# tue-mps/simple-tad

Measured on AMD Instinct MI355X. Metric: clips/sec (16x224^2 ViT-B) fwd+bwd, higher is better.
Workload: dtype bf16; 1 GPU; vit_base_patch16_224 16x224x224, 32 clips/GPU, fwd+bwd+AdamW fine-tune step with CE loss on synthetic labels (BASELINE configs[2]/[3]); global_batch=32, per_gpu_batch=32, parallelism=dp1, residual_stream=f32, operands=bf16, parameters=86228738

## Files before the change

simple_tad_amd/csrc/gemm.hip:

```cpp
#include <math.h>
#include <stdlib.h>
#include <string>
#include "common.h"

TAD_NAMESPACE_BEGIN

int launch_reduce_partials(const float* partial, float* out, int splits, int64_t n, int accumulate, hipStream_t st);
int launch_reduce_col_ranges(const float* partial, int N, int splits, int c0, float* out0, int c1, float* out1, int n, int accumulate,
                             hipStream_t st);
int launch_reduce_dw(const float* partial, float* out, int splits, int64_t n, int accumulate, const float* partial2, int rows2, int n2,
                     float* out2a, float* out2b, int n2a, int c2b, hipStream_t st);
int launch_reduce_dw_pair(const float* partial, float* outA, float* outB, int64_t nA, int splits, int64_t n, int accumulate, const float* partial2,
                          int rows2, int n2, float* out2a, float* out2b, int n2a, int c2b, hipStream_t st);

#ifdef TAD_GEMM_ABLATION
#define DBG_BITS(p) ((p).debug)
#else
#define DBG_BITS(p) 0
#endif

enum { EPI_PLAIN = 0, EPI_GELU = 1, EPI_RESIDUAL = 2, EPI_DGELU = 3, EPI_RESMOD = 4 };

struct GemmNT {
  const uint16_t* A;
  const uint16_t* B;
  void* C;
  const float* bias;
  const float* bias2;
  int bias_seg;
  float colscale;
  int colscale_cols;
  const float* residual;
  const float* gamma;
  const float* rowscale;
// ... 831 lines not shown
                                                 c_rs, ob, 0, ST_AUX);
        }
      }
    }
    if (q < 6) { STAMP(5 + 2 * q); }
    if (q + 1 < NCHUNK) lds_barrier();
  }
#undef DROP_CHUNK
  }
  STAMP(2);
#ifdef TAD_GEMM_ABLATION
  if (p.stamps) {
    asm volatile("s_waitcnt vmcnt(0)" ::: "memory");
    STAMP(3);
  }
  ++stamp_i;
#endif
  if (!has_next) break;
  if (!DIRECT) lds_barrier();
  }
}

struct GemmTN {
  const uint16_t* P;
  const uint16_t* Q;
  float* slab;
  float* bias_slab;
  int Mr, N, K;
  int rows_per_split;
  int debug;
  const uint16_t* P2;
  const uint16_t* Q2;
  int N1;
};

__device__ __forceinline__ int sw_tn(int row) { return ((row & 3) | ((row >> 1) & 4)) << 1; }


template <int BM, int BN, int WAVES_M, int WAVES_N, int STAGES, bool PDEEP = false>
__global__ __launch_bounds__(WAVES_M* WAVES_N * 64) void gemm_tn_kernel(const GemmTN p) {
  static_assert(!PDEEP || STAGES == 2, "PDEEP extends the two-stage ring");
  constexpr int BKT = BK;
  constexpr int NW = WAVES_M * WAVES_N;
  constexpr int WTM = BM / WAVES_M, WTN = BN / WAVES_N;
  constexpr int MREP = WTM / 16, NREP = WTN / 16;
  constexpr int PROW = BM * 2, QROW = BN * 2;
  constexpr int KSTEPS = BKT / 32;
  constexpr int P_BYTES = BKT * PROW, Q_BYTES = BKT * QROW;
  constexpr int STAGE_BYTES = P_BYTES + Q_BYTES;
  constexpr int P_PIECES = P_BYTES / 1024 / NW, Q_PIECES = Q_BYTES / 1024 / NW;
  constexpr int P_LPR = PROW / 16, Q_LPR = QROW / 16;
  static_assert(P_BYTES % (1024 * NW) == 0 && Q_BYTES % (1024 * NW) == 0, "tile must split into 1-KiB DMA pieces per wave");
  static_assert(P_LPR <= 64 && Q_LPR <= 64 && PROW >= 256 && QROW >= 256, "row length");
  constexpr int LOADS = P_PIECES + Q_PIECES;
  constexpr int LDS_BYTES_TN = PDEEP ? 3 * P_BYTES + 2 * Q_BYTES : STAGES * STAGE_BYTES;
  static_assert(LDS_BYTES_TN <= 160 * 1024, "LDS budget");
  __shared__ __attribute__((aligned(1024))) char lds[LDS_BYTES_TN];

  const int tid = threadIdx.x;
  const int lane = tid & 63;
  const int wave = __builtin_amdgcn_readfirstlane(tid >> 6);
  const int wm = wave / WAVES_N, wn = wave % WAVES_N;

  const int tiles_k = (p.K + BN - 1) / BN;
  const int tiles = tiles_k * ((p.N + BM - 1) / BM);
  const int lin = xcd_remap(blockIdx.x, gridDim.x);
// ... 161 lines not shown
      const int k = k0 + wn * WTN + 16 * j + 4 * g;
      if (n < p.N && k < p.K)
        *reinterpret_cast<float4*>(out + (int64_t)n * p.K + k) = make_float4(acc[i][j][0], acc[i][j][1], acc[i][j][2], acc[i][j][3]);
    }
  }
}

#ifndef TAD_GEMM_W4_TU

static int cu_count();

TAD_NAMESPACE_END
namespace tad { namespace knobs {
#ifndef TAD_OPND_F16
static int env_int(const char* name) {
  const char* v = getenv(name);
  return v ? atoi(v) : 0;
}
int gemm_debug = env_int("TAD_GEMM_DEBUG");
int nt_persist = !env_int("TAD_GEMM_NO_PERSIST");
int nt_direct = getenv("TAD_GEMM_DIRECT_EPI") ? env_int("TAD_GEMM_DIRECT_EPI") : 1;
int nt_split = getenv("TAD_GEMM_SPLIT_TAIL") ? env_int("TAD_GEMM_SPLIT_TAIL") : 1;
int nt_sk_defer = getenv("TAD_GEMM_SPLITK_DEFER") ? env_int("TAD_GEMM_SPLITK_DEFER") : 1;
int nt_splitk = getenv("TAD_GEMM_SPLITK_TAIL") ? env_int("TAD_GEMM_SPLITK_TAIL") : 1;
int nt_variant = env_int("TAD_GEMM_NT_VARIANT");
int nt_group_m_knob = getenv("TAD_GEMM_GROUP_M") ? env_int("TAD_GEMM_GROUP_M") : 0;
int tn_variant = env_int("TAD_GEMM_TN_VARIANT");
int nt_w4_plain = getenv("TAD_GEMM_W4_PLAIN") ? env_int("TAD_GEMM_W4_PLAIN") : 640;
int nt_w4_epilogues = getenv("TAD_GEMM_W4_EPILOGUES") ? env_int("TAD_GEMM_W4_EPILOGUES") : 4;
int tn_pair = getenv("TAD_GEMM_TN_PAIR") ? env_int("TAD_GEMM_TN_PAIR") : 1;
int nt_short_k = getenv("TAD_GEMM_SHORT_K") ? env_int("TAD_GEMM_SHORT_K") : 1;
int nt_tail_192 = getenv("TAD_GEMM_TAIL_192") ? env_int("TAD_GEMM_TAIL_192") : 1;
int tn_w4 = getenv("TAD_GEMM_TN_W4") ? env_int("TAD_GEMM_TN_W4") : 1;
int tn_pdeep = env_int("TAD_GEMM_TN_PDEEP");
unsigned long long* nt_stamps = nullptr;
long long nt_launches = 0;
#else
extern int gemm_debug, nt_persist, nt_direct, nt_split, nt_splitk, nt_variant, nt_group_m_knob, tn_variant, tn_pdeep, nt_sk_defer, tn_w4, nt_w4_plain, nt_w4_epilogues, nt_tail_192, nt_short_k, tn_pair;
extern unsigned long long* nt_stamps;
extern long long nt_launches;
#endif
}}
TAD_NAMESPACE_BEGIN
using namespace knobs;

static int nt_group_m(int tiles_m, int tiles_n, int K) {
  if (nt_group_m_knob > 0) return nt_group_m_knob;
  return K >= 2048 ? 4 : 8;
}


template <int EPI, bool OUT_BF16>
static void launch_nt_variant(int v, GemmNT& p, hipStream_t st) {
  auto tiles = [&](int bm, int bn) { return ((p.M + bm - 1) / bm) * ((p.N + bn - 1) / bn); };
  const int no_persist = !nt_persist;
  if (((EPI == EPI_RESIDUAL && OUT_BF16) || EPI == EPI_RESMOD) && (v == 1 || v == 7)) v = 3;
  if (v != 2 && v != 4 && v != 5 && p.rowscale && p.rows_per_scale < 256) v = 2;
  const int grid_p = cu_count() & ~7;
  const int bn = v == 1 ? 256 : 128;
  const bool persist = !no_persist && (v == 1 || v == 3) && grid_p >= 8 && tiles(256, bn) > grid_p + grid_p / 2;
  p.group_m = nt_group_m((p.M + 255) / 256, (p.N + bn - 1) / bn, p.K);
#define NT_LAUNCH(BM_, BN_, WM_, WN_, ST_, PER_, DIR_, GRID_, THREADS_)                                                              \
  hipLaunchKernelGGL((gemm_nt_kernel<BM_, BN_, WM_, WN_, ST_, EPI, OUT_BF16, PER_, DIR_>), dim3(GRID_), dim3(THREADS_), 0, st, p)
  const bool direct = nt_direct == 2 || (nt_direct == 1 && EPI == EPI_PLAIN && OUT_BF16);
  switch (v) {
    case 1:
      if constexpr (!(EPI == EPI_RESIDUAL && OUT_BF16) && EPI != EPI_RESMOD) {
        if (persist) { if (direct) NT_LAUNCH(256, 256, 2, 4, 2, true, true, grid_p, 512); else NT_LAUNCH(256, 256, 2, 4, 2, true, false, grid_p, 512); }
        else { if (direct) NT_LAUNCH(256, 256, 2, 4, 2, false, true, tiles(256, 256), 512); else NT_LAUNCH(256, 256, 2, 4, 2, false, false, tiles(256, 256), 512); }
      }
      break;
// ... 266 lines not shown
  return (K > 0 && pad256 * 3 >= pad128 * 4) ? 3 : 1;
}
static int cu_count() {
  static const int n = [] {
    int dev = 0, v = 0;
    if (hipGetDevice(&dev) != hipSuccess || hipDeviceGetAttribute(&v, hipDeviceAttributeMultiprocessorCount, dev) != hipSuccess || v <= 0) v = 256;
    return v;
  }();
  return n;
}
static int tn_plan(int64_t Mr, int N, int K, int* splits, int* rows_per_split) {
  const int bn = tn_variant(K) != 3 ? 256 : 128;
  const int tiles = ((N + 255) / 256) * ((K + bn - 1) / bn);
  const int64_t ktiles = (Mr + BK - 1) / BK;
  const int cus = cu_count();
  const double epi_units = 6.0;
  const double reduce_units = (double)N * (double)K * 8.0 / 4.0e12 / 2.0e-6;
  int best = 1;
  double best_cost = 1e300;
  for (int s = 1; s <= 64 && s <= ktiles; ++s) {
    const int64_t per = (ktiles + s - 1) / s;
    const int s_eff = (int)((ktiles + per - 1) / per);
    if (s_eff != s) continue;
    const int64_t rounds = ((int64_t)tiles * s + cus - 1) / cus;
    const double cost = (double)rounds * ((double)per + epi_units) + (s > 1 ? s * reduce_units : 0.0);
    if (cost < best_cost) { best_cost = cost; best = s; }
  }
  const int64_t per = (ktiles + best - 1) / best;
  *splits = best;
  *rows_per_split = (int)(per * BK);
  return tiles;
}

size_t gemm_tn_workspace_bytes(int64_t Mr, int N, int K) {
  int s, r;
  tn_plan(Mr, N, K, &s, &r);
  const int bn = tn_variant(K) != 3 ? 256 : 128;
  return (size_t)s * ((size_t)N * (size_t)K + (size_t)((K + bn - 1) / bn) * (size_t)N) * sizeof(float);
}

int launch_gemm_tn(const uint16_t* P, const uint16_t* Q, float* out, float* bias_out, float* bias_out2, int accumulate, void* ws,
                   size_t ws_bytes, int64_t Mr, int N, int K, hipStream_t st) {
  if (const int rc = sk_check_pending_error()) return rc;
  if (!(Mr > 0 && N > 0 && K > 0)) { set_error("gemm_tn: empty problem"); return TAD_EINVAL; }
  if (N % 8 || K % 8) { set_error("gemm_tn: N=%d and K=%d must be multiples of 8", N, K); return TAD_EINVAL; }
  if (Mr * (int64_t)N * 2 >= (1ll << 32) || Mr * (int64_t)K * 2 >= (1ll << 32)) { set_error("gemm_tn: operand exceeds 4 GiB"); return TAD_EINVAL; }
  GemmTN p{};
  p.P = P; p.Q = Q; p.slab = (float*)ws; p.Mr = (int)Mr; p.N = N; p.K = K;
  p.debug = gemm_debug;
  int splits;
  const int tiles = tn_plan(Mr, N, K, &splits, &p.rows_per_split);
  const int tiles_k = (K + (tn_variant(K) != 3 ? 256 : 128) - 1) / (tn_variant(K) != 3 ? 256 : 128);
  if (ws_bytes < (size_t)splits * ((size_t)N * K + (size_t)tiles_k * N) * sizeof(float)) { set_error("gemm_tn: workspace too small"); return TAD_ENOSPACE; }
  p.bias_slab = bias_out ? p.slab + (size_t)splits * N * K : nullptr;
  if (tn_variant(K) == 1 && knobs::tn_w4 && !knobs::tn_pdeep && p.rows_per_split >= 2 * BK && !p.debug) {
    const int rc = launch_gemm_tn_w4(p, tiles * splits, st);
    if (rc) return rc;
  } else if (tn_variant(K) == 1 && knobs::tn_pdeep)
    hipLaunchKernelGGL((gemm_tn_kernel<256, 256, 2, 4, 2, true>), dim3(tiles * splits), dim3(512), 0, st, p);
  else if (tn_variant(K) == 1)
    hipLaunchKernelGGL((gemm_tn_kernel<256, 256, 2, 4, 2>), dim3(tiles * splits), dim3(512), 0, st, p);
  else
    hipLaunchKernelGGL((gemm_tn_kernel<256, 128, 4, 2, 3>), dim3(tiles * splits), dim3(512), 0, st, p);
  int rc = check_launch("gemm_tn");
  if (rc) return rc;
  if (!bias_out) return launch_reduce_partials(p.slab, out, splits, (int64_t)N * K, accumulate, st);
  if (bias_out2) return launch_reduce_dw(p.slab, out, splits, (int64_t)N * K, accumulate, p.bias_slab, splits * tiles_k, N, bias_out, bias_out2, N / 3, 2 * (N / 3), st);
  return launch_reduce_dw(p.slab, out, splits, (int64_t)N * K, accumulate, p.bias_slab, splits * tiles_k, N, bias_out, nullptr, N, 0, st);
}

int launch_gemm_tn_pair(const uint16_t* P1, const uint16_t* Q1, float* out1, float* bias_out1, float* bias_out1b, int N1, const uint16_t* P2,
                        const uint16_t* Q2, float* out2, int N2, int accumulate, void* ws, size_t ws_bytes, int64_t Mr, int K, hipStream_t st) {
  if (const int rc = sk_check_pending_error()) return rc;
  if (!(Mr > 0 && N1 > 0 && N2 > 0 && K > 0)) { set_error("gemm_tn_pair: empty problem"); return TAD_EINVAL; }
  if (N1 % 8 || N2 % 8 || K % 8) { set_error("gemm_tn_pair: N1=%d, N2=%d and K=%d must be multiples of 8", N1, N2, K); return TAD_EINVAL; }
  const int N = N1 + N2;
  int splits = 0, rows_per_split = 0;
  const int tiles = tn_plan(Mr, N, K, &splits, &rows_per_split);
  const int tiles_k = (K + 255) / 256;
  const bool fits = tn_pair && tn_variant(K) == 1 && knobs::tn_w4 && !knobs::tn_pdeep && !gemm_debug && N1 % 256 == 0 && rows_per_split >= 2 * BK &&
                    Mr * (int64_t)N * 2 < (1ll << 32) && Mr * (int64_t)K * 2 < (1ll << 32) &&
                    ws_bytes >= (size_t)splits * ((size_t)N * K + (size_t)tiles_k * N) * sizeof(float);
  if (!fits) {
    const int rc = launch_gemm_tn(P1, Q1, out1, bias_out1, bias_out1b, accumulate, ws, ws_bytes, Mr, N1, K, st);
    if (rc) return rc;
    return launch_gemm_tn(P2, Q2, out2, nullptr, nullptr, accumulate, ws, ws_bytes, Mr, N2, K, st);
  }
  GemmTN p{};
  p.P = P1; p.Q = Q1; p.P2 = P2; p.Q2 = Q2; p.N1 = N1;
  p.slab = (float*)ws; p.Mr = (int)Mr; p.N = N; p.K = K; p.rows_per_split = rows_per_split;
  p.bias_slab = bias_out1 ? p.slab + (size_t)splits * N * K : nullptr;
  int rc = launch_gemm_tn_w4(p, tiles * splits, st);
  if (rc) return rc;
  const int64_t n1 = (int64_t)N1 * K, n = (int64_t)N * K;
  if (!bias_out1) return launch_reduce_dw_pair(p.slab, out1, out2, n1, splits, n, accumulate, nullptr, 0, 0, nullptr, nullptr, 0, 0, st);
  if (bias_out1b) return launch_reduce_dw_pair(p.slab, out1, out2, n1, splits, n, accumulate, p.bias_slab, splits * tiles_k, N, bias_out1, bias_out1b, N1 / 3, 2 * (N1 / 3), st);
  return launch_reduce_dw_pair(p.slab, out1, out2, n1, splits, n, accumulate, p.bias_slab, splits * tiles_k, N, bias_out1, nullptr, N1, 0, st);
}

TAD_NAMESPACE_END

using namespace tad;

extern "C" {

int tad_linear_fwd(const uint16_t* x, const uint16_t* w, const float* bias, void* y, int y_dtype, int epilogue, uint16_t* preact,
                   const float* residual, const float* gamma, const float* rowscale, int rows_per_scale, void* ws, size_t ws_bytes,
                   int64_t M, int N, int K, tad_stream_t stream) {
  TAD_REQUIRE(x && w && y, "linear_fwd: null pointer");
  TAD_REQUIRE(y_dtype == TAD_F32 || y_dtype == TAD_OP16, "linear_fwd: bad y_dtype %d", y_dtype);
  TAD_REQUIRE(epilogue >= TAD_EPI_BIAS && epilogue <= TAD_EPI_BIAS_RESIDUAL, "linear_fwd: bad epilogue %d", epilogue);
  TAD_REQUIRE(!rowscale || rows_per_scale > 0, "linear_fwd: rows_per_scale must be positive");
  TAD_REQUIRE(M > 0 && M < (1ll << 31), "linear_fwd: bad M");
  GemmNT p{};
  p.A = x; p.B = w; p.C = y; p.bias = bias; p.c_bf16 = (y_dtype == TAD_OP16);
  p.M = (int)M; p.N = N; p.K = K;
  p.rows_per_scale = rows_per_scale > 0 ? rows_per_scale : 1;
  if (epilogue == TAD_EPI_BIAS_GELU) { p.epi = EPI_GELU; p.preact = preact; }
  else if (epilogue == TAD_EPI_BIAS_RESIDUAL) { p.epi = EPI_RESIDUAL; p.residual = residual; p.gamma = gamma; p.rowscale = rowscale; }
  else p.epi = EPI_PLAIN;
  return launch_gemm_nt(p, (hipStream_t)stream, ws, ws ? ws_bytes : 0);
}

#ifndef TAD_OPND_F16
// ... 38 lines not shown
int tad_linear_bwd_weight_qkv(const uint16_t* dy, const uint16_t* x, float* dW, float* dq_bias, float* dv_bias, int accumulate, void* ws,
                              size_t ws_bytes, int64_t M, int N, int K, tad_stream_t stream) {
  TAD_REQUIRE(dy && x && dW && ws && dq_bias && dv_bias, "linear_bwd_weight_qkv: null pointer");
  TAD_REQUIRE(N > 0 && N % 12 == 0, "linear_bwd_weight_qkv: N=%d must be 3 x a multiple of 4", N);
  return launch_gemm_tn(dy, x, dW, dq_bias, dv_bias, accumulate, ws, ws_bytes, M, N, K, (hipStream_t)stream);
}

int tad_linear_bwd_weight_pair(const uint16_t* dy1, const uint16_t* x1, float* dW1, float* db1, float* db1b, int N1, const uint16_t* dy2,
                               const uint16_t* x2, float* dW2, int N2, int accumulate, void* ws, size_t ws_bytes, int64_t M, int K, tad_stream_t stream) {
  TAD_REQUIRE(dy1 && x1 && dW1 && dy2 && x2 && dW2 && ws, "linear_bwd_weight_pair: null pointer");
  TAD_REQUIRE(!db1b || db1, "linear_bwd_weight_pair: db1b (the v_bias third) comes with db1 (the q_bias third)");
  TAD_REQUIRE(!db1b || (N1 > 0 && N1 % 12 == 0), "linear_bwd_weight_pair: N1=%d must be 3 x a multiple of 4 for the split bias sums", N1);
  TAD_REQUIRE(((uintptr_t)dW1 | (uintptr_t)dW2 | (uintptr_t)db1 | (uintptr_t)db1b) % 16 == 0, "linear_bwd_weight_pair: dW1, dW2, db1 and db1b must be 16-byte aligned");
  return launch_gemm_tn_pair(dy1, x1, dW1, db1, db1b, N1, dy2, x2, dW2, N2, accumulate, ws, ws_bytes, M, K, (hipStream_t)stream);
}

#ifndef TAD_OPND_F16
int tad_linear_tuning(const char* key, int value) {
  TAD_REQUIRE(key, "linear_tuning: null key");
  const std::string k(key);
  if (k == "splitk_tail") { TAD_REQUIRE(value >= 0 && value <= 2, "linear_tuning: splitk_tail=%d not in {0, 1, 2}", value); nt_splitk = value; return TAD_OK; }
  if (k == "persistent") nt_persist = value != 0;
  else if (k == "direct_epilogue") { TAD_REQUIRE(value >= 0 && value <= 2, "linear_tuning: direct_epilogue=%d not in 0..2", value); nt_direct = value; }
  else if (k == "debug") gemm_debug = value;
  else if (k == "group_m") { TAD_REQUIRE(value >= 0 && value <= 1024, "linear_tuning: group_m=%d out of range", value); nt_group_m_knob = value; }
  else if (k == "variant") { TAD_REQUIRE(value >= 0 && value <= 9 && value != 6, "linear_tuning: variant=%d not one of 0..5, 7, 8, 9", value); nt_variant = value; }
  else if (k == "splitk_defer") { TAD_REQUIRE(value == 0 || value == 1, "linear_tuning: splitk_defer=%d not in {0, 1}", value); nt_sk_defer = value; }
  else if (k == "tn_pair") { TAD_REQUIRE(value == 0 || value == 1, "linear_tuning: tn_pair=%d not in {0, 1}", value); tn_pair = value; }
  else if (k == "short_k") { TAD_REQUIRE(value == 0 || value == 1, "linear_tuning: short_k=%d not in {0, 1}", value); nt_short_k = value; }
  else if (k == "tail_192") { TAD_REQUIRE(value == 0 || value == 1, "linear_tuning: tail_192=%d not in {0, 1}", value); nt_tail_192 = value; }
  else if (k == "w4_epilogues") { TAD_REQUIRE(value >= 0 && value < 16, "linear_tuning: w4_epilogues=%d not a mask of bits 1..3", value); nt_w4_epilogues = value; }
  else if (k == "w4_plain") { TAD_REQUIRE(value >= 0, "linear_tuning: w4_plain=%d must be >= 0", value); nt_w4_plain = value; }
  else if (k == "tn_w4") { TAD_REQUIRE(value == 0 || value == 1, "linear_tuning: tn_w4=%d not in {0, 1}", value); tn_w4 = value; }
  else if (k == "tn_pdeep") { TAD_REQUIRE(value == 0 || value == 1, "linear_tuning: tn_pdeep=%d not in {0, 1}", value); tn_pdeep = value; }
  else if (k == "split_tail") { TAD_REQUIRE(value >= 0 && value <= 2, "linear_tuning: split_tail=%d not in 0..2", value); nt_split = value; }
  else { set_error("linear_tuning: unknown key '%s'", key); return TAD_EINVAL; }
  return TAD_OK;
}

int tad_linear_tuning_get(const char* key, int* value) {
  TAD_REQUIRE(key && value, "linear_tuning_get: null pointer");
  const std::string k(key);
  const struct { const char* name; const int* v; } table[] = {
      {"splitk_tail", &nt_splitk}, {"persistent", &nt_persist}, {"direct_epilogue", &nt_direct}, {"debug", &gemm_debug}, {"group_m", &nt_group_m_knob},
      {"variant", &nt_variant}, {"splitk_defer", &nt_sk_defer}, {"tn_pair", &tn_pair}, {"short_k", &nt_short_k}, {"tail_192", &nt_tail_192},
      {"w4_epilogues", &nt_w4_epilogues}, {"w4_plain", &nt_w4_plain}, {"tn_w4", &tn_w4}, {"tn_pdeep", &tn_pdeep}, {"split_tail", &nt_split}};
  for (const auto& e : table)
    if (k == e.name) { *value = *e.v; return TAD_OK; }
  set_error("linear_tuning_get: unknown key '%s'", key);
  return TAD_EINVAL;
}

long long tad_linear_kernel_launches(void) { return nt_launches; }

int tad_linear_debug_stamps(void* buf) {
#ifndef TAD_GEMM_ABLATION
  if (buf) { set_error("linear_debug_stamps: timeline stamps need an ablation build (TAD_BUILD_ABLATION=1 python -m simple_tad_amd.build --force)"); return TAD_EINVAL; }
#endif
  nt_stamps = (unsigned long long*)buf;
  return TAD_OK;
}
#endif

int tad_linear_bwd_input(const uint16_t* dy, const uint16_t* wT, void* dx, int dx_dtype, const uint16_t* gelu_preact, void* ws, size_t ws_bytes,
                         int64_t M, int N, int K, tad_stream_t stream) {
  TAD_REQUIRE(dy && wT && dx, "linear_bwd_input: null pointer");
  TAD_REQUIRE(dx_dtype == TAD_F32 || dx_dtype == TAD_OP16, "linear_bwd_input: bad dx_dtype %d", dx_dtype);
  TAD_REQUIRE(M > 0 && M < (1ll << 31), "linear_bwd_input: bad M");
  GemmNT p{};
  p.A = dy; p.B = wT; p.C = dx; p.c_bf16 = (dx_dtype == TAD_OP16);
  p.M = (int)M; p.N = K; p.K = N;
  p.rows_per_scale = 1;
  p.epi = gelu_preact ? EPI_DGELU : EPI_PLAIN;
  p.dgelu_h = gelu_preact;
  return launch_gemm_nt(p, (hipStream_t)stream, ws, ws ? ws_bytes : 0);
}

#ifndef TAD_OPND_F16
size_t tad_linear_bwd_weight_workspace_bytes(int64_t M, int N, int K) {
// ... 53 lines not shown
```

simple_tad_amd/csrc/gemm_w4.hip:

```cpp
#define TAD_GEMM_W4_TU
#include "gemm.hip"

__device__ __forceinline__ void mfma_16x16x32_vgpr(f32x4& d, const op16x8& a, const op16x8& b) {
#ifdef TAD_OPND_F16
  asm volatile("s_nop 1\n\tv_mfma_f32_16x16x32_f16 %0, %1, %2, %0\n\ts_nop 3" : "+v"(d) : "v"(a), "v"(b));
#else
  asm volatile("s_nop 1\n\tv_mfma_f32_16x16x32_bf16 %0, %1, %2, %0\n\ts_nop 3" : "+v"(d) : "v"(a), "v"(b));
#endif
}

#ifndef TNW4_ABL_NO_DMA
#define TNW4_ABL_NO_DMA 0
#endif
#ifndef TNW4_ABL_NO_READS
#define TNW4_ABL_NO_READS 0
#endif
#ifndef TNW4_ABL_NO_SYNC
#define TNW4_ABL_NO_SYNC 0
#endif
#ifndef TNW4_2BAR
#define TNW4_2BAR 1
#endif
#ifndef TNW4_DMA_GROUPS
#define TNW4_DMA_GROUPS 8
#endif
__global__ __launch_bounds__(256, 1) void gemm_tn_w4_kernel(const GemmTN p) {
  constexpr int NW = 4, BM = 256, BN = 256, PROW = BM * 2, QROW = BN * 2, P_BYTES = BK * PROW, Q_BYTES = BK * QROW, STAGE_BYTES = P_BYTES + Q_BYTES;
  static_assert(STAGE_BYTES == 65536 && PROW == 512, "slot toggle = bit 16 of the LDS address");
  __shared__ __attribute__((aligned(1024))) char lds[2 * STAGE_BYTES];
  const int tid = threadIdx.x, lane = tid & 63;
  const int wave = __builtin_amdgcn_readfirstlane(tid >> 6);
  const int wm = wave >> 1, wn = wave & 1;
  const int tiles_k = (p.K + BN - 1) / BN;
  const int tiles = tiles_k * ((p.N + BM - 1) / BM);
  const int lin = xcd_remap(blockIdx.x, gridDim.x);
  const int split = lin / tiles;
  const int tile = lin - split * tiles;
  const int tn_ = tile / tiles_k, tk_ = tile - tn_ * tiles_k;
  const int n0 = tn_ * BM, k0 = tk_ * BN;
  const int mr0 = split * p.rows_per_split;
  const int nt = p.rows_per_split / BK;
  const bool seg2 = p.N1 > 0 && n0 >= p.N1;
  const uint16_t* const Pg = seg2 ? p.P2 : p.P;
  const uint16_t* const Qg = seg2 ? p.Q2 : p.Q;
  const int ldp = p.N1 > 0 ? (seg2 ? p.N - p.N1 : p.N1) : p.N;
  const int np0 = seg2 ? n0 - p.N1 : n0;
  const int p_bytes = (int)((int64_t)p.Mr * ldp * 2), q_bytes = (int)((int64_t)p.Mr * p.K * 2);
  uint32_t p_off[8], q_off[8];
#pragma unroll
  for (int i = 0; i < 8; ++i) {
    const int row = (i * NW + wave) * 2 + (lane >> 5);
    const int chunk = (lane & 31) ^ sw_tn(row);
    int col = np0 + chunk * 8;
    if (col > ldp - 8) col = ldp - 8;
    p_off[i] = (uint32_t)(mr0 + row) * (uint32_t)(ldp * 2) + (uint32_t)(col * 2);
    col = k0 + chunk * 8;
    if (col > p.K - 8) col = p.K - 8;
    q_off[i] = (uint32_t)(mr0 + row) * (uint32_t)(p.K * 2) + (uint32_t)(col * 2);
  }
#define TNW4_PIECE(SLOT, idx, t_)                                                                                                            \
  if ((idx) < 8) w4_dma_piece(Pg, p_bytes, lds + (SLOT) + (((idx) & 7) * NW + wave) * 1024, p_off[(idx) & 7], (uint32_t)(t_) * BK * (uint32_t)(ldp * 2)); \
  else w4_dma_piece(Qg, q_bytes, lds + (SLOT) + P_BYTES + (((idx) & 7) * NW + wave) * 1024, q_off[(idx) & 7], (uint32_t)(t_) * BK * (uint32_t)(p.K * 2))
  const int g = lane >> 4, li = lane & 15;
  uint32_t p_rd[8], q_rd[8];
  {
    const int r0 = 8 * g + (li >> 2);
    const uint32_t l0 = lds_addr(lds);
#pragma unroll
    for (int i = 0; i < 8; ++i) {
      const int cp = wm * 128 + 16 * (i ^ wn) + 4 * (li & 3), cq = wn * 128 + 16 * i + 4 * (li & 3);
      p_rd[i] = l0 + (uint32_t)(r0 * PROW + (((cp >> 3) ^ sw_tn(r0)) << 4) + (cp & 7) * 2);
// ... 70 lines not shown
    }
    static_for<0, 8>([&](auto gc) {
      constexpr int i = decltype(gc)::value;
      if constexpr (NEXT2) {
        if constexpr (TNW4_2BAR) {
          if constexpr (!TNW4_ABL_NO_DMA) { TNW4_PIECE(slot, TNW4_K1IDX(i), t + 2); }
        } else if constexpr (i < TNW4_DMA_GROUPS && !TNW4_ABL_NO_DMA) {
          static_for<0, 16 / TNW4_DMA_GROUPS>([&](auto pc) {
            constexpr int piece = i * (16 / TNW4_DMA_GROUPS) + decltype(pc)::value;
            TNW4_PIECE(slot, piece, t + 2);
          });
        }
      }
      if constexpr (NEXT && !TNW4_ABL_NO_READS) { TNW4_READ(0, 0, i); }
      const op16x8 pf = join_tr(pl[1][i], ph[1][i]);
#pragma unroll
      for (int j = 0; j < 8; ++j) acc[i][j] = TAD_MFMA_16x16x32(join_tr(ql[1][j], qh[1][j]), pf, acc[i][j]);
      __builtin_amdgcn_sched_barrier(0);
    });
    if (bias_now) {
#pragma unroll
      for (int ib = 0; ib < 4; ++ib) mfma_16x16x32_vgpr(bacc[ib], join_tr(pl[1][2 * ib], ph[1][2 * ib]), ones);
    }
    slot ^= STAGE_BYTES;
  };
  int t = 0;
  for (; t + 2 < nt; ++t) tn_tile(std::true_type{}, std::true_type{}, t);
  tn_tile(std::true_type{}, std::false_type{}, t);
  tn_tile(std::false_type{}, std::false_type{}, t + 1);
#undef TNW4_PIECE
#undef TNW4_READ

  asm volatile("s_nop 15\n\ts_nop 15" : "+v"(bacc[0]), "+v"(bacc[1]), "+v"(bacc[2]), "+v"(bacc[3])::"memory");
  if (bias_on && li == 0) {
    float* bo = p.bias_slab + ((int64_t)split * tiles_k + tk_) * p.N;
#pragma unroll
    for (int ib = 0; ib < 4; ++ib)
#pragma unroll
      for (int r = 0; r < 4; ++r) {
        const int n = n0 + wm * 128 + 16 * (ib * 2 + wn) + 4 * g + r;
        if (n < p.N) bo[n] = bacc[ib][r];
      }
  }
  float* out = p.slab + (int64_t)split * p.N * p.K;
#pragma unroll
  for (int i = 0; i < 8; ++i) {
    const int n = n0 + wm * 128 + 16 * (i ^ wn) + li;
#pragma unroll
    for (int j = 0; j < 8; ++j) {
      const int k = k0 + wn * 128 + 16 * j + 4 * g;
      if (n < p.N && k < p.K)
        *reinterpret_cast<float4*>(out + (int64_t)n * p.K + k) = make_float4(acc[i][j][0], acc[i][j][1], acc[i][j][2], acc[i][j][3]);
    }
  }
}

int launch_gemm_tn_w4(const GemmTN& p, int grid, hipStream_t st) {
  hipLaunchKernelGGL(gemm_tn_w4_kernel, dim3(grid), dim3(256), 0, st, p);
  return check_launch("gemm_tn_w4");
}

int launch_gemm_nt_w4(const GemmNT& p, int grid_persist, hipStream_t st) {
  const int tiles = ((p.M + 255) / 256) * ((p.N + 255) / 256);
#define W4_LAUNCH(E, O)                                                                                                          \
  do {                                                                                                                           \
    if (grid_persist > 0) hipLaunchKernelGGL((gemm_nt_kernel<256, 256, 2, 2, 2, E, O, true, false>), dim3(grid_persist), dim3(256), 0, st, p); \
    else hipLaunchKernelGGL((gemm_nt_kernel<256, 256, 2, 2, 2, E, O, false, false>), dim3(tiles), dim3(256), 0, st, p);        \
  } while (0)
  switch (p.epi) {
    case EPI_PLAIN: if (p.c_bf16) W4_LAUNCH(EPI_PLAIN, true); else W4_LAUNCH(EPI_PLAIN, false); break;
    case EPI_GELU: if (p.c_bf16) W4_LAUNCH(EPI_GELU, true); else W4_LAUNCH(EPI_GELU, false); break;
    case EPI_DGELU: if (p.c_bf16) W4_LAUNCH(EPI_DGELU, true); else W4_LAUNCH(EPI_DGELU, false); break;
    case EPI_RESIDUAL:
      if (p.c_bf16) { set_error("gemm_nt (4-wave): no 16-bit residual epilogue"); return TAD_EINVAL; }
      W4_LAUNCH(EPI_RESIDUAL, false);
      break;
    default: set_error("gemm_nt (4-wave): no kernel for epilogue %d", p.epi); return TAD_EINVAL;
  }
#undef W4_LAUNCH
  return check_launch("gemm_nt_w4");
}

TAD_NAMESPACE_END
```

simple_tad_amd/kernels.py:

```python
from __future__ import annotations

import ctypes as C
from typing import Optional

import torch

from . import _lib
from ._lib import EPI_BIAS, EPI_BIAS_GELU, EPI_BIAS_RESIDUAL, TAD_BF16, TAD_F16, TAD_F32, check

_workspaces = {}


class LaunchProfiler:

    def __init__(self, only=None, stride=1):
        self.items = []
        self.only = set(only) if only else None
        self.stride = max(1, int(stride))
        self.seen = {}

    def wants(self, kernel):
        if self.only is not None and kernel not in self.only:
            return False
        n = self.seen.get(kernel, 0)
# ... 369 lines not shown
        assert tuple(residual.shape) == (M, N)
    y = torch.empty((M, N), dtype=out_dtype, device=x.device)
    pre = torch.empty((M, N), dtype=op, device=x.device) if want_preact else None
    ws, wsb = _linear_ws(M, N, K, x.device)
    with _timed("gemm_nt", 2.0 * M * N * K, 2.0 * (M * K + N * K) + y.element_size() * M * N + (4.0 * M * N if residual is not None else 0.0)
                + (2.0 * M * N if want_preact else 0.0)):
        check(_fn("tad_linear_fwd", op)(x.data_ptr(), w.data_ptr(), _p(bias), y.data_ptr(), _dt(y), epilogue, _p(pre), _p(residual),
                                         _p(gamma), _p(rowscale), int(rows_per_scale), ws, wsb, M, N, K, _stream()), "tad_linear_fwd")
    return y, pre


_linear_splitk = True


def set_linear_splitk(on: bool):
    global _linear_splitk
    _linear_splitk = bool(on)


def _linear_ws(M, N, K, device):
    if not _linear_splitk:
        return None, 0
    nbytes = _lib.load().tad_linear_workspace_bytes(M, N, K)
    if not nbytes:
        return None, 0
    return linear_workspace(nbytes, device).data_ptr(), nbytes


def _pad_reduction(a, b, mult: int = 64):
    pad = (-a.shape[1]) % mult
    return torch.nn.functional.pad(a, (0, pad)).contiguous(), torch.nn.functional.pad(b, (0, pad)).contiguous()


LINEAR_TUNING_DEFAULTS = dict(persistent=1, direct_epilogue=1, split_tail=1, splitk_tail=1, group_m=0, variant=0, tn_pdeep=0, splitk_defer=1, tn_w4=1, w4_plain=640, w4_epilogues=4, tail_192=1, short_k=1, tn_pair=1)


def linear_workspace(nbytes: int, device) -> torch.Tensor:
    key = _ws_key(device)
    ent = _workspaces.get(key)
    if ent is None:
        ent = _workspaces[key] = {"ws": None, "retired": []}
    buf = ent.get("lin")
    if buf is None or buf.numel() < nbytes:
        if buf is not None:
            ent["retired"].append(buf)
        buf = torch.empty(nbytes, dtype=torch.uint8, device=device)
        ent["lin"] = buf
    return buf


def linear_kernel_launches() -> int:
    return int(_lib.load().tad_linear_kernel_launches())


def linear_tuning(**knobs):
    for k, v in knobs.items():
        check(_lib.load().tad_linear_tuning(k.encode(), int(v)), f"tad_linear_tuning({k}={v})")


def linear_tuning_get(key: str) -> int:
    v = C.c_int(0)
    check(_lib.load().tad_linear_tuning_get(key.encode(), C.byref(v)), f"tad_linear_tuning_get({key})")
    return int(v.value)


def linear_bwd_input(dy, wT, out_dtype=None, gelu_preact=None):
    op = _req16(dy, "linear_bwd_input.dy")
# ... 466 lines not shown
```

Before: 728.8 clips/sec.

## Add in-kernel split-K reduction and N-fast rasterization to TN weight-gradient GEMM

Adds an optional path where each split of the TN w4 GEMM writes its partial and bumps a tagged per-tile counter. The last arriving block sums all splits (and bias partials) into the output, which removes the separate reduce kernel launch and its extra pass over memory. The fused path is gated off by default. It also adds a default-on tile rasterization that iterates N tiles fastest when K tiles outnumber N tiles, to change operand reuse across concurrently running blocks. The fused path adds atomic counters, fences and a serialized tail reduction in the last block.

Measured after the change: 728.4 clips/sec, median of 2. Within noise of the previous version (-0.1%).

```diff
diff --git a/simple_tad_amd/csrc/gemm.hip b/simple_tad_amd/csrc/gemm.hip
--- a/simple_tad_amd/csrc/gemm.hip
+++ b/simple_tad_amd/csrc/gemm.hip
@@ -1,5 +1,6 @@
 #include <math.h>
 #include <stdlib.h>
+#include <atomic>
 #include <string>
 #include "common.h"
 
@@ -897,6 +898,15 @@
   const uint16_t* P2;
   const uint16_t* Q2;
   int N1;
+  int raster;
+  unsigned long long* cnt;
+  unsigned long long tag;
+  float* out;
+  float* outB;
+  float* bias_out;
+  float* bias_out2;
+  int n2a, c2b;
+  int splits, accumulate;
 };
 
 __device__ __forceinline__ int sw_tn(int row) { return ((row & 3) | ((row >> 1) & 4)) << 1; }
@@ -1124,11 +1134,13 @@
 int nt_short_k = getenv("TAD_GEMM_SHORT_K") ? env_int("TAD_GEMM_SHORT_K") : 1;
 int nt_tail_192 = getenv("TAD_GEMM_TAIL_192") ? env_int("TAD_GEMM_TAIL_192") : 1;
 int tn_w4 = getenv("TAD_GEMM_TN_W4") ? env_int("TAD_GEMM_TN_W4") : 1;
+int tn_fused_reduce = env_int("TAD_GEMM_TN_FUSED_REDUCE");
+int tn_raster = getenv("TAD_GEMM_TN_RASTER") ? env_int("TAD_GEMM_TN_RASTER") : 1;
 int tn_pdeep = env_int("TAD_GEMM_TN_PDEEP");
 unsigned long long* nt_stamps = nullptr;
 long long nt_launches = 0;
 #else
-extern int gemm_debug, nt_persist, nt_direct, nt_split, nt_splitk, nt_variant, nt_group_m_knob, tn_variant, tn_pdeep, nt_sk_defer, tn_w4, nt_w4_plain, nt_w4_epilogues, nt_tail_192, nt_short_k, tn_pair;
+extern int gemm_debug, nt_persist, nt_direct, nt_split, nt_splitk, nt_variant, nt_group_m_knob, tn_variant, tn_pdeep, nt_sk_defer, tn_w4, tn_fused_reduce, tn_raster, nt_w4_plain, nt_w4_epilogues, nt_tail_192, nt_short_k, tn_pair;
 extern unsigned long long* nt_stamps;
 extern long long nt_launches;
 #endif
@@ -1461,11 +1473,33 @@
   return tiles;
 }
 
+static size_t tn_counter_bytes(int N, int K) {
+  const size_t tiles_n = (size_t)(N + 255) / 256;
+  return (tiles_n * (size_t)((K + 255) / 256) + tiles_n) * sizeof(unsigned long long);
+}
+
 size_t gemm_tn_workspace_bytes(int64_t Mr, int N, int K) {
   int s, r;
   tn_plan(Mr, N, K, &s, &r);
   const int bn = tn_variant(K) != 3 ? 256 : 128;
-  return (size_t)s * ((size_t)N * (size_t)K + (size_t)((K + bn - 1) / bn) * (size_t)N) * sizeof(float);
+  return (size_t)s * ((size_t)N * (size_t)K + (size_t)((K + bn - 1) / bn) * (size_t)N) * sizeof(float) + tn_counter_bytes(N, K);
+}
+
+static bool tn_fuse(GemmTN& p, int splits, int tiles_k, void* ws, size_t ws_bytes) {
+#ifdef TAD_OPND_F16
+  static std::atomic<unsigned long long> launches{1ull << 62};
+#else
+  static std::atomic<unsigned long long> launches{0};
+#endif
+  const size_t slab_bytes = (size_t)splits * ((size_t)p.N * p.K + (size_t)tiles_k * p.N) * sizeof(float);
+  if (!knobs::tn_fused_reduce || (int64_t)p.N * p.K * 4 >= (1ll << 31) || (int64_t)splits * tiles_k >= 65536 || ws_bytes < slab_bytes + tn_counter_bytes(p.N, p.K)) return false;
+  p.cnt = reinterpret_cast<unsigned long long*>((char*)ws + slab_bytes);
+  unsigned long long z = (launches.fetch_add(1, std::memory_order_relaxed) + 1) * 0x9E3779B97F4A7C15ull;
+  z = (z ^ (z >> 30)) * 0xBF58476D1CE4E5B9ull;
+  z = (z ^ (z >> 27)) * 0x94D049BB133111EBull;
+  p.tag = (z ^ (z >> 31)) >> 16;
+  p.splits = splits;
+  return true;
 }
 
 int launch_gemm_tn(const uint16_t* P, const uint16_t* Q, float* out, float* bias_out, float* bias_out2, int accumulate, void* ws,
@@ -1480,9 +1514,15 @@
   int splits;
   const int tiles = tn_plan(Mr, N, K, &splits, &p.rows_per_split);
   const int tiles_k = (K + (tn_variant(K) != 3 ? 256 : 128) - 1) / (tn_variant(K) != 3 ? 256 : 128);
-  if (ws_bytes < (size_t)splits * ((size_t)N * K + (size_t)tiles_k * N) * sizeof(float)) { set_error("gemm_tn: workspace too small"); return TAD_ENOSPACE; }
+  if (ws_bytes < gemm_tn_workspace_bytes(Mr, N, K)) { set_error("gemm_tn: workspace too small"); return TAD_ENOSPACE; }
   p.bias_slab = bias_out ? p.slab + (size_t)splits * N * K : nullptr;
   if (tn_variant(K) == 1 && knobs::tn_w4 && !knobs::tn_pdeep && p.rows_per_split >= 2 * BK && !p.debug) {
+    p.raster = knobs::tn_raster;
+    if (tn_fuse(p, splits, tiles_k, ws, ws_bytes)) {
+      p.out = out; p.accumulate = accumulate;
+      p.bias_out = bias_out; p.bias_out2 = bias_out2; p.n2a = bias_out2 ? N / 3 : N; p.c2b = bias_out2 ? 2 * (N / 3) : 0;
+      return launch_gemm_tn_w4(p, tiles * splits, st);
+    }
     const int rc = launch_gemm_tn_w4(p, tiles * splits, st);
     if (rc) return rc;
   } else if (tn_variant(K) == 1 && knobs::tn_pdeep)
@@ -1509,7 +1549,7 @@
   const int tiles_k = (K + 255) / 256;
   const bool fits = tn_pair && tn_variant(K) == 1 && knobs::tn_w4 && !knobs::tn_pdeep && !gemm_debug && N1 % 256 == 0 && rows_per_split >= 2 * BK &&
                     Mr * (int64_t)N * 2 < (1ll << 32) && Mr * (int64_t)K * 2 < (1ll << 32) &&
-                    ws_bytes >= (size_t)splits * ((size_t)N * K + (size_t)tiles_k * N) * sizeof(float);
+                    ws_bytes >= gemm_tn_workspace_bytes(Mr, N, K);
   if (!fits) {
     const int rc = launch_gemm_tn(P1, Q1, out1, bias_out1, bias_out1b, accumulate, ws, ws_bytes, Mr, N1, K, st);
     if (rc) return rc;
@@ -1519,6 +1559,12 @@
   p.P = P1; p.Q = Q1; p.P2 = P2; p.Q2 = Q2; p.N1 = N1;
   p.slab = (float*)ws; p.Mr = (int)Mr; p.N = N; p.K = K; p.rows_per_split = rows_per_split;
   p.bias_slab = bias_out1 ? p.slab + (size_t)splits * N * K : nullptr;
+  p.raster = knobs::tn_raster;
+  if (tn_fuse(p, splits, tiles_k, ws, ws_bytes)) {
+    p.out = out1; p.outB = out2; p.accumulate = accumulate;
+    p.bias_out = bias_out1; p.bias_out2 = bias_out1b; p.n2a = bias_out1b ? N1 / 3 : N1; p.c2b = bias_out1b ? 2 * (N1 / 3) : 0;
+    return launch_gemm_tn_w4(p, tiles * splits, st);
+  }
   int rc = launch_gemm_tn_w4(p, tiles * splits, st);
   if (rc) return rc;
   const int64_t n1 = (int64_t)N1 * K, n = (int64_t)N * K;
@@ -1623,6 +1669,8 @@
   else if (k == "w4_epilogues") { TAD_REQUIRE(value >= 0 && value < 16, "linear_tuning: w4_epilogues=%d not a mask of bits 1..3", value); nt_w4_epilogues = value; }
   else if (k == "w4_plain") { TAD_REQUIRE(value >= 0, "linear_tuning: w4_plain=%d must be >= 0", value); nt_w4_plain = value; }
   else if (k == "tn_w4") { TAD_REQUIRE(value == 0 || value == 1, "linear_tuning: tn_w4=%d not in {0, 1}", value); tn_w4 = value; }
+  else if (k == "tn_fused_reduce") { TAD_REQUIRE(value == 0 || value == 1, "linear_tuning: tn_fused_reduce=%d not in {0, 1}", value); tn_fused_reduce = value; }
+  else if (k == "tn_raster") { TAD_REQUIRE(value == 0 || value == 1, "linear_tuning: tn_raster=%d not in {0, 1}", value); tn_raster = value; }
   else if (k == "tn_pdeep") { TAD_REQUIRE(value == 0 || value == 1, "linear_tuning: tn_pdeep=%d not in {0, 1}", value); tn_pdeep = value; }
   else if (k == "split_tail") { TAD_REQUIRE(value >= 0 && value <= 2, "linear_tuning: split_tail=%d not in 0..2", value); nt_split = value; }
   else { set_error("linear_tuning: unknown key '%s'", key); return TAD_EINVAL; }
@@ -1635,7 +1683,7 @@
   const struct { const char* name; const int* v; } table[] = {
       {"splitk_tail", &nt_splitk}, {"persistent", &nt_persist}, {"direct_epilogue", &nt_direct}, {"debug", &gemm_debug}, {"group_m", &nt_group_m_knob},
       {"variant", &nt_variant}, {"splitk_defer", &nt_sk_defer}, {"tn_pair", &tn_pair}, {"short_k", &nt_short_k}, {"tail_192", &nt_tail_192},
-      {"w4_epilogues", &nt_w4_epilogues}, {"w4_plain", &nt_w4_plain}, {"tn_w4", &tn_w4}, {"tn_pdeep", &tn_pdeep}, {"split_tail", &nt_split}};
+      {"w4_epilogues", &nt_w4_epilogues}, {"w4_plain", &nt_w4_plain}, {"tn_w4", &tn_w4}, {"tn_fused_reduce", &tn_fused_reduce}, {"tn_raster", &tn_raster}, {"tn_pdeep", &tn_pdeep}, {"split_tail", &nt_split}};
   for (const auto& e : table)
     if (k == e.name) { *value = *e.v; return TAD_OK; }
   set_error("linear_tuning_get: unknown key '%s'", key);
diff --git a/simple_tad_amd/csrc/gemm_w4.hip b/simple_tad_amd/csrc/gemm_w4.hip
--- a/simple_tad_amd/csrc/gemm_w4.hip
+++ b/simple_tad_amd/csrc/gemm_w4.hip
@@ -7,6 +7,22 @@
 #else
   asm volatile("s_nop 1\n\tv_mfma_f32_16x16x32_bf16 %0, %1, %2, %0\n\ts_nop 3" : "+v"(d) : "v"(a), "v"(b));
 #endif
+}
+
+constexpr uint32_t TN_OOB = 0x80000000u;
+__device__ __forceinline__ bool tn_arrive(unsigned long long* w, unsigned long long tag, uint32_t total) {
+  unsigned long long old = __hip_atomic_load(w, __ATOMIC_RELAXED, __HIP_MEMORY_SCOPE_AGENT);
+  for (;;) {
+    const unsigned long long now = ((old >> 16) == tag ? old : tag << 16) + 1;
+    if (__hip_atomic_compare_exchange_strong(w, &old, now, __ATOMIC_RELAXED, __ATOMIC_RELAXED, __HIP_MEMORY_SCOPE_AGENT)) {
+      if ((uint32_t)(now & 0xffff) != total) return false;
+      __hip_atomic_store(w, 0ull, __ATOMIC_RELAXED, __HIP_MEMORY_SCOPE_AGENT);
+      return true;
+    }
+  }
+}
+__device__ __forceinline__ u32x4 tn_load_share(const float* share, int bytes, uint32_t off) {
+  return __builtin_amdgcn_raw_buffer_load_b128(__builtin_amdgcn_make_buffer_rsrc((void*)share, 0, bytes, 0x00020000), off, 0, 0);
 }
 
 #ifndef TNW4_ABL_NO_DMA
@@ -36,7 +52,9 @@
   const int lin = xcd_remap(blockIdx.x, gridDim.x);
   const int split = lin / tiles;
   const int tile = lin - split * tiles;
-  const int tn_ = tile / tiles_k, tk_ = tile - tn_ * tiles_k;
+  const int tiles_n = tiles / tiles_k;
+  const bool n_fast = p.raster && tiles_k > tiles_n;
+  const int tn_ = n_fast ? tile % tiles_n : tile / tiles_k, tk_ = n_fast ? tile / tiles_n : tile - tn_ * tiles_k;
   const int n0 = tn_ * BM, k0 = tk_ * BN;
   const int mr0 = split * p.rows_per_split;
   const int nt = p.rows_per_split / BK;
@@ -173,6 +191,7 @@
 #undef TNW4_READ
 
   asm volatile("s_nop 15\n\ts_nop 15" : "+v"(bacc[0]), "+v"(bacc[1]), "+v"(bacc[2]), "+v"(bacc[3])::"memory");
+  const bool fused = p.cnt != nullptr;
   if (bias_on && li == 0) {
     float* bo = p.bias_slab + ((int64_t)split * tiles_k + tk_) * p.N;
 #pragma unroll
@@ -180,18 +199,113 @@
 #pragma unroll
       for (int r = 0; r < 4; ++r) {
         const int n = n0 + wm * 128 + 16 * (ib * 2 + wn) + 4 * g + r;
-        if (n < p.N) bo[n] = bacc[ib][r];
+        if (n < p.N) {
+          if (fused) __hip_atomic_store(reinterpret_cast<uint32_t*>(bo + n), __float_as_uint(bacc[ib][r]), __ATOMIC_RELAXED, __HIP_MEMORY_SCOPE_AGENT);
+          else bo[n] = bacc[ib][r];
+        }
       }
   }
   float* out = p.slab + (int64_t)split * p.N * p.K;
-#pragma unroll
-  for (int i = 0; i < 8; ++i) {
-    const int n = n0 + wm * 128 + 16 * (i ^ wn) + li;
-#pragma unroll
-    for (int j = 0; j < 8; ++j) {
-      const int k = k0 + wn * 128 + 16 * j + 4 * g;
-      if (n < p.N && k < p.K)
-        *reinterpret_cast<float4*>(out + (int64_t)n * p.K + k) = make_float4(acc[i][j][0], acc[i][j][1], acc[i][j][2], acc[i][j][3]);
+  if (!fused) {
+#pragma unroll
+    for (int i = 0; i < 8; ++i) {
+      const int n = n0 + wm * 128 + 16 * (i ^ wn) + li;
+#pragma unroll
+      for (int j = 0; j < 8; ++j) {
+        const int k = k0 + wn * 128 + 16 * j + 4 * g;
+        if (n < p.N && k < p.K)
+          *reinterpret_cast<float4*>(out + (int64_t)n * p.K + k) = make_float4(acc[i][j][0], acc[i][j][1], acc[i][j][2], acc[i][j][3]);
+      }
+    }
+    return;
+  }
+  {
+    const auto slab_rs = __builtin_amdgcn_make_buffer_rsrc((void*)out, 0, p.N * p.K * 4, 0x00020000);
+#pragma unroll
+    for (int i = 0; i < 8; ++i) {
+      const int n = n0 + wm * 128 + 16 * (i ^ wn) + li;
+#pragma unroll
+      for (int j = 0; j < 8; ++j) {
+        const int k = k0 + wn * 128 + 16 * j + 4 * g;
+        __builtin_amdgcn_raw_buffer_store_b128(__builtin_bit_cast(u32x4, acc[i][j]), slab_rs, (n < p.N && k < p.K) ? (uint32_t)(n * p.K + k) * 4u : TN_OOB, 0, 16);
+      }
+    }
+  }
+  asm volatile("s_waitcnt vmcnt(0)" ::: "memory");
+  __syncthreads();
+  int* const last_lds = reinterpret_cast<int*>(lds);
+  if (tid == 0) {
+    int last = 0;
+    if (tn_arrive(p.cnt + tn_ * tiles_k + tk_, p.tag, (uint32_t)p.splits)) last |= 1;
+    if (bias_on && tn_arrive(p.cnt + tiles + tn_, p.tag, (uint32_t)(p.splits * tiles_k))) last |= 2;
+    if (last) {
+      __builtin_amdgcn_fence(__ATOMIC_ACQUIRE, "agent");
+      asm volatile("s_waitcnt vmcnt(0)" ::: "memory");
+    }
+    *last_lds = last;
+  }
+  __syncthreads();
+  const int last = __builtin_amdgcn_readfirstlane(*last_lds);
+  if (last & 2) {
+    const int n = n0 + tid;
+    const int rows2 = p.splits * tiles_k;
+    float* dst = nullptr;
+    if (n < p.n2a) dst = p.bias_out + n;
+    else if (p.bias_out2 && n >= p.c2b && n < p.c2b + p.n2a) dst = p.bias_out2 + (n - p.c2b);
+    if (dst) {
+      const float* src = p.slab + (int64_t)p.splits * p.N * p.K + n;
+      float s = 0.f;
+      int r = 0;
+      for (; r + 8 <= rows2; r += 8) {
+        float v[8];
+#pragma unroll
+        for (int q = 0; q < 8; ++q) v[q] = src[(int64_t)(r + q) * p.N];
+#pragma unroll
+        for (int q = 0; q < 8; ++q) s += v[q];
+      }
+      for (; r < rows2; ++r) s += src[(int64_t)r * p.N];
+      if (p.accumulate) s += *dst;
+      *dst = s;
+    }
+  }
+  if (!(last & 1)) return;
+  {
+    constexpr int TN_RB = 4;
+    const int64_t share_elems = (int64_t)p.N * p.K;
+    const int rows_d = p.N1 > 0 ? (seg2 ? p.N - p.N1 : p.N1) : p.N;
+    float* const dbase = seg2 ? p.outB : p.out;
+    const auto in_rs = __builtin_amdgcn_make_buffer_rsrc((void*)p.slab, 0, p.N * p.K * 4, 0x00020000);
+    const auto out_rs = __builtin_amdgcn_make_buffer_rsrc((void*)dbase, 0, rows_d * p.K * 4, 0x00020000);
+    const int k = k0 + 4 * (tid & 63);
+    const int S = p.splits;
+    for (int r0 = tid >> 6; r0 < BM; r0 += 4 * TN_RB) {
+      uint32_t off_in[TN_RB], off_out[TN_RB];
+      f32x4 s[TN_RB];
+#pragma unroll
+      for (int b = 0; b < TN_RB; ++b) {
+        const int r = r0 + 4 * b;
+        const bool live = n0 + r < p.N && k < p.K;
+        off_in[b] = live ? (uint32_t)((n0 + r) * p.K + k) * 4u : TN_OOB;
+        off_out[b] = live ? (uint32_t)((np0 + r) * p.K + k) * 4u : TN_OOB;
+        s[b] = __builtin_bit_cast(f32x4, __builtin_amdgcn_raw_buffer_load_b128(in_rs, off_in[b], 0, 0));
+      }
+#pragma unroll 2
+      for (int sh = 1; sh < S; ++sh) {
+        f32x4 v[TN_RB];
+#pragma unroll
+        for (int b = 0; b < TN_RB; ++b) v[b] = __builtin_bit_cast(f32x4, tn_load_share(p.slab + sh * share_elems, p.N * p.K * 4, off_in[b]));
+#pragma unroll
+        for (int b = 0; b < TN_RB; ++b) s[b] += v[b];
+      }
+      if (p.accumulate) {
+        f32x4 o[TN_RB];
+#pragma unroll
+        for (int b = 0; b < TN_RB; ++b) o[b] = __builtin_bit_cast(f32x4, __builtin_amdgcn_raw_buffer_load_b128(out_rs, off_out[b], 0, 0));
+#pragma unroll
+        for (int b = 0; b < TN_RB; ++b) s[b] += o[b];
+      }
+#pragma unroll
+      for (int b = 0; b < TN_RB; ++b) __builtin_amdgcn_raw_buffer_store_b128(__builtin_bit_cast(u32x4, s[b]), out_rs, off_out[b], 0, 0);
     }
   }
 }
diff --git a/simple_tad_amd/kernels.py b/simple_tad_amd/kernels.py
--- a/simple_tad_amd/kernels.py
+++ b/simple_tad_amd/kernels.py
@@ -425,7 +425,7 @@
     return torch.nn.functional.pad(a, (0, pad)).contiguous(), torch.nn.functional.pad(b, (0, pad)).contiguous()
 
 
-LINEAR_TUNING_DEFAULTS = dict(persistent=1, direct_epilogue=1, split_tail=1, splitk_tail=1, group_m=0, variant=0, tn_pdeep=0, splitk_defer=1, tn_w4=1, w4_plain=640, w4_epilogues=4, tail_192=1, short_k=1, tn_pair=1)
+LINEAR_TUNING_DEFAULTS = dict(persistent=1, direct_epilogue=1, split_tail=1, splitk_tail=1, group_m=0, variant=0, tn_pdeep=0, splitk_defer=1, tn_w4=1, tn_fused_reduce=0, tn_raster=1, w4_plain=640, w4_epilogues=4, tail_192=1, short_k=1, tn_pair=1)
 
 
 def linear_workspace(nbytes: int, device) -> torch.Tensor:
```
